# zhiqiangdon/pose-adv-aug

Hardware: AMD Instinct MI355X
Metric: images/sec, 2-stack HG 256x256 bs=24 per GPU, full training step (higher is better)
Workload: dtype bf16; 1 GPU; BASELINE configs[1]: 2-stack hourglass chan 256, bs=24/GPU, 256x256 MPII-shape synthetic frames (720x1280 uint8 resident in HBM), on-device HumanAug warp, heat-map MSE, RMSprop, PCKh; global_batch=24, parallelism=dp1, ranks_seen=1, devices_seen=1

## Files before the change

### include/poseadv.h

```cpp
#ifndef POSEADV_H
#define POSEADV_H
#include <stddef.h>
#include <stdint.h>
#ifdef __cplusplus
extern "C" {
#endif

const char* pa_last_error(void);
int pa_version(void);
int pa_dtype(void);
float pa_grad_scale(void);


int pa_gaussian_heatmap(const double* pts, float* out, int B, int J, int H, int W, void* stream);

int pa_weighted_l2(const float* pred, const float* gt, const float* weight, size_t n, float* loss, void* stream);
int pa_weighted_l2_grad(const float* pred, const float* gt, const float* weight, size_t n, const float* gout_dev,
                        float* dpred, void* stream);

int pa_get_preds(const float* maps, int B, int J, int H, int W, float* preds, float* maxval, void* stream);

int pa_final_preds(const float* maps, const float* center, const float* scale, const float* rot,
                   int B, int J, int H, int W, float* out, float* scratch_preds, void* stream);

// ... 157 lines not shown

int pa_asn_forward(pa_net* asn, pa_net* pose, int train, float* logits_scale, float* logits_rot);
const float* pa_asn_probs(const pa_net* asn);
int pa_asn_backward(pa_net* asn, pa_net* pose, const float* target_scale, const float* target_rot, float* loss);
int pa_asn_set_log_eps(pa_net* asn, float eps);

int pa_asn_forward_masks(pa_net* asn, pa_net* pose, int train, float* mask_logits);
int pa_asn_backward_masks(pa_net* asn, pa_net* pose, const float* dlogits);
int pa_hg_set_dropout_masks(pa_net* net, const float* masks);

int pa_hg_accuracy(pa_net* net, int stack, const int32_t* idxs, int nidx, float* acc, float* scratch);

int pa_hg_pckh(pa_net* net, int stack, const float* center, const float* scale, const float* rot, const float* gt_pts,
               const float* norm, const int32_t* idxs, int nidx, float* acc, float* person, float* scratch);

int pa_net_meters_async(pa_net* net, int on);

#define PA_PROF_CLASSES 12
int pa_net_profile_begin(pa_net* net);
int pa_net_profile_report(pa_net* net, double* out_host, int cap_classes, int* n_classes);
int pa_net_profile_classes(const pa_net* net, int32_t* out_host, int cap);
int pa_net_set_fin_prologue(pa_net* net, int max_rows);
int pa_net_set_pool_route(pa_net* net, int on);
int pa_net_design_bytes(const pa_net* net, double* out_host);
int pa_copy_probe(void* dst, const void* src, size_t bytes, void* stream);
int pa_copy_probe_form(void* dst, const void* src, size_t bytes, int form, void* stream);
int pa_conv2d_time(int mode, int variant, int B, int Cin, int Cout, int H, int W, int k, int iters, void* ws, float* ms_out, void* stream);
int pa_conv_plan_describe(int B, int H, int W, int Cin, int Cout, int taps, int in_mode, int add1_mode, int add2_mode, int ep_mode,
                          int ep2_mode, int fin_rows, int flags, int cus, int* out, int cap);
int pa_conv_launch_log(int* out, int cap);

int pa_net_set_multi_stream(pa_net* net, int on);

int pa_hg_debug_tensor(pa_net* net, const char* which, int grad, float* out, int* shape4);

int pa_asn_debug_tensor(pa_net* net, const char* which, int grad, float* out, int* shape4);

#ifdef __cplusplus
}
#endif
#endif
```

### pose_adv_aug_amd/_lib.py

```python
import ctypes as C
import os

import torch

_HERE = os.path.dirname(os.path.abspath(__file__))
DTYPE = os.environ.get('POSEADV_DTYPE', 'bf16').lower()
if DTYPE not in ('bf16', 'fp16'):
    raise ValueError('POSEADV_DTYPE must be bf16 or fp16')
LIB_PATH = os.path.join(_HERE, 'libposeadv_hip.so' if DTYPE == 'bf16' else 'libposeadv_hip_fp16.so')


def set_dtype(name):
    global DTYPE, LIB_PATH
    name = name.lower()
    if name not in ('bf16', 'fp16'):
        raise ValueError('dtype must be bf16 or fp16')
    if _lib is not None and name != DTYPE:
        raise PoseAdvError('the %s library is already loaded in this process' % DTYPE)
    DTYPE = name
    LIB_PATH = os.path.join(_HERE, 'libposeadv_hip.so' if name == 'bf16' else 'libposeadv_hip_fp16.so')


def act_dtype():
    return torch.bfloat16 if DTYPE == 'bf16' else torch.float16
# ... 115 lines not shown
    'pa_hg_bucket_wait': (_i, [_vp, _i, _vp]),
    'pa_hg_train_step': (_i, [_vp, _vp, _vp, _i, _i, _vp]),
    'pa_hg_set_loss_total': (_i, [_vp, _vp]),
    'pa_hg_set_heat_grads': (_i, [_vp, C.POINTER(_vp), _i]),
    'pa_hg_set_image_grad': (_i, [_vp, _vp, _i]),
    'pa_stem_dgrad_workspace_bytes': (_sz, [_i, _i, _i]),
    'pa_stem_dgrad': (_i, [_vp, _vp, _vp, _i, _i, _i, _i, _vp, _vp]),
    'pa_hg_accuracy': (_i, [_vp, _i, _vp, _i, _vp, _vp]),
    'pa_hg_forward_half': (_i, [_vp, _vp, _vp, _i]),
    'pa_asn_forward': (_i, [_vp, _vp, _i, _vp, _vp]),
    'pa_asn_probs': (_vp, [_vp]),
    'pa_asn_backward': (_i, [_vp, _vp, _vp, _vp, _vp]),
    'pa_asn_set_log_eps': (_i, [_vp, _f]),
    'pa_hg_pckh': (_i, [_vp, _i, _vp, _vp, _vp, _vp, _vp, _vp, _i, _vp, _vp, _vp]),
    'pa_net_meters_async': (_i, [_vp, _i]),
    'pa_net_profile_begin': (_i, [_vp]),
    'pa_net_profile_report': (_i, [_vp, C.POINTER(C.c_double), _i, C.POINTER(_i)]),
    'pa_net_design_bytes': (_i, [_vp, C.POINTER(C.c_double)]),
    'pa_copy_probe': (_i, [_vp, _vp, _sz, _vp]),
    'pa_copy_probe_form': (_i, [_vp, _vp, _sz, _i, _vp]),
    'pa_params_csr': (_i, [_vp, _i, _vp, _vp]),
    'pa_net_set_fin_prologue': (_i, [_vp, _i]),
    'pa_net_set_pool_route': (_i, [_vp, _i]),
    'pa_wgrad_group_workspace_bytes': (_sz, [_vp, _i]),
    'pa_wgrad_group': (_i, [_vp, _i, _i, _vp, _vp]),
    'pa_conv2d_time': (_i, [_i] * 9 + [_vp, C.POINTER(C.c_float), _vp]),
    'pa_conv_plan_describe': (_i, [_i] * 14 + [C.POINTER(_i), _i]),
    'pa_conv_launch_log': (_i, [C.POINTER(_i), _i]),
    'pa_net_profile_classes': (_i, [_vp, C.POINTER(C.c_int32), _i]),
    'pa_net_set_multi_stream': (_i, [_vp, _i]),
    'pa_hg_debug_tensor': (_i, [_vp, C.c_char_p, _i, _vp, C.POINTER(_i)]),
    'pa_asn_debug_tensor': (_i, [_vp, C.c_char_p, _i, _vp, C.POINTER(_i)]),
}

EXPORTS = sorted(_PROTOS)


def lib():
    global _lib
    if _lib is None:
        if not os.path.isfile(LIB_PATH):
            raise PoseAdvError('%s not found: run `python -c "import __graft_entry__ as g; g.build()"` '
                               '(there is no CPU fallback)' % LIB_PATH)
        try:
            l = C.CDLL(LIB_PATH)
        except OSError as e:
# ... 41 lines not shown
```

### pose_adv_aug_amd/csrc/api.hip

```cpp
#include "../../include/poseadv.h"
#include "net.h"
#include "warp_bwd.h"
#include "soft_argmax.h"
#include <stdio.h>
#include <string.h>
#include <new>
#include <string>

static thread_local char g_err[1024] = "";
void pa_set_error(const char* what, hipError_t e, const char* file, int line) {
    snprintf(g_err, sizeof g_err, "%s:%d: %s -> %s", file, line, what, hipGetErrorString(e));
}
void pa_set_error_msg(const char* msg) { snprintf(g_err, sizeof g_err, "%s", msg); }

struct pa_net { Net n; };
#define ST(s) reinterpret_cast<hipStream_t>(s)
#define TRY(x) do { int _r = (x); if (_r) { if (!g_err[0]) pa_set_error("kernel launch", (hipError_t)_r, __FILE__, __LINE__); return _r; } } while (0)
#define NEED_PTR(fn, p) do { if (!(p)) { pa_set_error_msg(fn ": " #p " is NULL"); return 1; } } while (0)
#define NEED_POS(fn, v) do { if ((v) < 1) { pa_set_error_msg(fn ": " #v " must be >= 1"); return 1; } } while (0)

extern "C" {

const char* pa_last_error(void) { return g_err; }
float pa_grad_scale(void) { return PA_GRAD_SCALE; }
// ... 874 lines not shown
}

int pa_net_profile_begin(pa_net* net) { net->n.prof.used = 0; net->n.prof.on = true; return 0; }
int pa_net_profile_report(pa_net* net, double* out, int cap_classes, int* n_classes) {
    net->n.prof.on = false;
    double full[PA_PROF_NCLS * 4];
    int r = net->n.prof.report(full);
    if (r) { pa_set_error("profile report", (hipError_t)r, __FILE__, __LINE__); return r; }
    for (int c = 0; c < PA_PROF_NCLS && c < cap_classes; ++c)
        for (int j = 0; j < 4; ++j) out[c * 4 + j] = full[c * 4 + j];
    if (n_classes) *n_classes = PA_PROF_NCLS;
    return 0;
}
int pa_net_set_fin_prologue(pa_net* net, int max_rows) {
    net->n.fin_rows_max = max_rows < 0 ? 0 : (max_rows > PA_FIN_SMALL_ROWS ? PA_FIN_SMALL_ROWS : max_rows);
    net->n.release_graph();
    return 0;
}
int pa_net_set_pool_route(pa_net* net, int on) {
    net->n.pool_route = on ? 3 : 0;
    net->n.release_graph();
    return 0;
}
int pa_net_design_bytes(const pa_net* net, double* out) { out[0] = net->n.dbytes_rd; out[1] = net->n.dbytes_wr; return 0; }

int pa_net_profile_classes(const pa_net* net, int32_t* out, int cap) {
    const std::vector<int>& q = net->n.prof.last_seq;
    for (int i = 0; i < cap && i < (int)q.size(); ++i) out[i] = q[i];
    return (int)q.size();
}

int pa_net_set_multi_stream(pa_net* net, int on) {
    if (net->n.ensure_streams()) return 1;
    net->n.release_graph();
    net->n.multi_stream = on != 0 && net->n.side != nullptr;
    return 0;
}

static int debug_copy(Net& n, const Act& a, int grad, float* out, int* shape4, const char* who, const bf16* mat) {
    if (grad < 0 || grad > 4) { pa_set_error_msg((std::string(who) + ": grad must be 0 .. 4").c_str()); return 1; }
    if ((grad == 1 || grad == 3) && !a.grad) { pa_set_error_msg((std::string(who) + ": this tensor has no gradient buffer").c_str()); return 1; }
    if (grad == 4 && !mat) { pa_set_error_msg((std::string(who) + ": no stored BatchNorm-backward gradient of this tensor in this step").c_str()); return 1; }
    shape4[0] = a.B; shape4[1] = a.C; shape4[2] = a.H; shape4[3] = a.W;
    if (!out) return 0;
    const PaOperand src = grad == 0 ? n.op(a) : grad == 1 ? pa_plain(a.grad) : grad == 2 ? pa_plain(a.raw) : grad == 3 ? n.gradop(a) : pa_plain(mat);
    TRY(pa_launch_nhwc_bf16_to_nchw_f32(src, out, a.B, a.C, a.H, a.W, n.st));
// ... 97 lines not shown
```

### pose_adv_aug_amd/csrc/asn.hip

```cpp
#include "net.h"
#include <string.h>

#define TRY(x) do { int _r = (x); if (_r) return _r; } while (0)

static PaEpilogue ep_plain() { PaEpilogue e; memset(&e, 0, sizeof e); e.mode = PA_OUT_PLAIN; return e; }

__global__ void pooladd_fwd_kernel(PaOperand hi, PaOperand lo, bf16* out, int B, int H, int W, int C) {
    const int CG = C / 8;
    const size_t total = (size_t)B * H * W * CG;
    for (size_t t = (size_t)blockIdx.x * blockDim.x + threadIdx.x; t < total; t += (size_t)gridDim.x * blockDim.x) {
        const int cg = (int)(t % CG);
        const size_t p = t / CG;
        const int x = (int)(p % W);
        const size_t q = p / W;
        const int y = (int)(q % H), b = (int)(q / H);
        const int c = cg * 8;
        float m[8], v[8];
#pragma unroll
        for (int k = 0; k < 4; ++k) {
            const size_t idx = (((size_t)b * 2 * H + 2 * y + (k >> 1)) * 2 * W + 2 * x + (k & 1)) * C + c;
            pa_read8(hi, idx, c, v);
#pragma unroll
            for (int j = 0; j < 8; ++j) m[j] = (k == 0) ? v[j] : fmaxf(m[j], v[j]);
        }
// ... 136 lines not shown
    for (int k = 0; k < 5; ++k) asn_in[k].declare(*this, names[k], chan, chan, false);
    char buf[32];
    for (int k = 0; k < 4; ++k) { snprintf(buf, sizeof buf, "merge%d.", k + 1); asn_merge[k].declare(*this, buf, chan, chan, false); }
    for (int k = 0; k < 3; ++k) { snprintf(buf, sizeof buf, "deep_merge.%d.", k); asn_deep[k].declare(*this, buf, chan, chan, false); }
    if (asn_dropout) {
        p_oc_w = add_param("out_conv.weight", {1, chan, 1, 1});
        p_oc_b = add_param("out_conv.bias", {1});
    } else {
        p_fcs_w = add_param("fc_scale.weight", {scale_num, chan});
        p_fcs_b = add_param("fc_scale.bias", {scale_num});
        p_fcr_w = add_param("fc_rotation.weight", {rot_num, chan});
        p_fcr_b = add_param("fc_rotation.bias", {rot_num});
    }
    n_params = (n_params + 3) & ~(size_t)3;
}

size_t Net::layout_asn(char* base) {
    Arena a; a.base = base;
    loss_dev = a.get<float>(64);
    a.take(0);
    stats_arena = base ? reinterpret_cast<float*>(base) : nullptr;
    stats_arena_floats = a.off / sizeof(float);
    prep_jobs = a.get<PaPrepJob>(convs.size());
    red_jobs = a.get<PaWgradReduceJob>(convs.size());
    bneval_jobs = a.get<PaBnEvalJob>(bns.size());
    const int H = res / 4;
    for (int k = 0; k < 5; ++k) asn_in[k].layout(*this, a, B, H >> k, H >> k, true);
    for (int k = 0; k < 4; ++k) {
        asn_pa[k] = new_act(a, B, H >> (k + 1), H >> (k + 1), chan, nullptr, true);
        asn_merge[k].layout(*this, a, B, H >> (k + 1), H >> (k + 1), true);
    }
    for (int k = 0; k < 3; ++k) asn_deep[k].layout(*this, a, B, H >> 4, H >> 4, true);
    asn_feat = a.get<float>((size_t)B * chan);
    asn_logits = a.get<float>((size_t)B * (asn_dropout ? 16 : scale_num + rot_num));
    asn_probs = a.get<float>((size_t)B * (scale_num + rot_num));
    asn_dlogits = a.get<float>((size_t)B * (scale_num + rot_num));
    a.take(0);
    return a.off;
}

int Net::forward_half(const float* img_nchw, const bf16* img4_in, bool train) {
    train_bn = train;
    TRY(ensure_streams());
    TRY(begin_step());
    if (!train) TRY(pa_launch_bn_eval(bneval_jobs, n_bneval, eps, st));
    const bf16* image = img4_in ? img4_in : img4;
// ... 110 lines not shown
```

### pose_adv_aug_amd/csrc/elementwise.hip

```cpp
#include "common.h"
#include "kernels.h"
#ifndef PA_ELT_PRIO
#define PA_ELT_PRIO 2
#endif
#define PA_SET_ELT_PRIO() do { if (PA_ELT_PRIO > 0) __builtin_amdgcn_s_setprio(PA_ELT_PRIO); } while (0)
#include "bn_fin.h"
#include <type_traits>
#include <hip/hip_ext.h>
static unsigned fin_launch_flags() { return pa_tuning().fin_anyorder ? hipExtAnyOrderLaunch : 0u; }
template <class... P, class... A>
static void fin_launch(void (*kernel)(P...), dim3 grid, int threads, hipStream_t st, A... args) {
    if (fin_launch_flags()) hipExtLaunchKernelGGL(kernel, grid, dim3(threads), 0, st, nullptr, nullptr, fin_launch_flags(), static_cast<P>(args)...);
    else hipLaunchKernelGGL(kernel, grid, dim3(threads), 0, st, static_cast<P>(args)...);
}

template <class F>
static void fin_dispatch(F f) {
    f(std::integral_constant<int, 512>{}, std::integral_constant<int, 8>{});
}
template <int FT, int FC>
__device__ __forceinline__ void reduce_partial_rows(const float* part, int rows, int C, int c0, float (*sums)[2]) {
    constexpr int SL = FT / FC;
    __shared__ __attribute__((aligned(16))) float red[SL][FC + 1][2];
    const int cl = threadIdx.x % FC, sl = threadIdx.x / FC;
// ... 1135 lines not shown
        const bool ok = n < j.Cout && c < j.Cin;
        const float* src = j.w + ((size_t)n * j.Cin + c) * j.taps;
        for (int tap = 0; tap < j.taps; ++tap) {
            const bf16 v = (bf16)(ok ? src[tap] : 0.f);
            j.wf[((size_t)n * j.taps + tap) * j.pad_cin + c] = v;
            tile[tap][tn][tc] = v;
        }
        __syncthreads();
        if (j.wb) {
            for (int tap = 0; tap < j.taps; ++tap)
                j.wb[((size_t)(c0 + tn) * j.taps + (j.taps - 1 - tap)) * j.pad_cout + n0 + tc] = tile[tap][tc][tn];
        }
        __syncthreads();
    }
}

int pa_launch_weight_prep(const PaPrepJob* jobs_dev, int njobs, int max_elems, hipStream_t st) {
    if (njobs <= 0) return 0;
    (void)max_elems;
    hipLaunchKernelGGL(weight_prep_kernel, dim3(32, njobs), dim3(1024), 0, st, jobs_dev);
    return (int)hipGetLastError();
}

__global__ void nchw_to_nhwc4_kernel(const float* src, bf16* dst, int B, int H, int W) {
    const size_t total = (size_t)B * H * W;
    for (size_t p = (size_t)blockIdx.x * blockDim.x + threadIdx.x; p < total; p += (size_t)gridDim.x * blockDim.x) {
        size_t hw = (size_t)H * W;
        size_t b = p / hw, r = p - b * hw;
        bf16x4 o;
        o[0] = (bf16)src[(b * 3 + 0) * hw + r];
        o[1] = (bf16)src[(b * 3 + 1) * hw + r];
        o[2] = (bf16)src[(b * 3 + 2) * hw + r];
        o[3] = (bf16)0.f;
        *reinterpret_cast<bf16x4*>(dst + p * 4) = o;
    }
}

int pa_launch_nchw_to_nhwc4(const float* src, bf16* dst, int B, int H, int W, hipStream_t st) {
    size_t total = (size_t)B * H * W;
    const int blocks = pa_grid_for(total, 256, 4096);
    hipLaunchKernelGGL(nchw_to_nhwc4_kernel, dim3(blocks), dim3(256), 0, st, src, dst, B, H, W);
    return (int)hipGetLastError();
}

__global__ void nhwc_to_nchw_f32_kernel(const float* src, float* dst, int B, int H, int W, int C) {
    const size_t total = (size_t)B * C * H * W;
// ... 137 lines not shown
```

### pose_adv_aug_amd/csrc/kernels.h

```cpp
#pragma once
#include "common.h"
#include "bn_fin.h"
#include "launch_plan.h"
#include "wgrad_plan.h"
#include "conv_plan.h"

struct PaConvArgs {
    PaOperand in;
    const bf16* w;
    const float* bias;
    PaOperand add1;
    PaOperand add2;
    PaEpilogue ep;
    bf16* out;
    int B, H, W, Cin, Cout, taps;
    bf16* dz_out;
    PaBnFin fin;
    int low_prio;
    int dbg;
    int xcd;
    PaEpilogue ep2;
    bf16* out2;
};
int pa_conv_cus();
// ... 68 lines not shown
    int B, Hm, Wm, layout;
    float scale;
};
int pa_launch_stem_dgrad(const PaStemDgradArgs& a, hipStream_t st);
int pa_launch_stem_pack(const float* w, bf16* wf, hipStream_t st);

int pa_launch_rmsprop(float* p, const float* g, float* v, size_t n, float lr, float alpha, float eps, float gscale, int* state, hipStream_t st);
struct PaRmspropOpts { float lr, alpha, eps, mom, wd; };
int pa_launch_rmsprop_opts(const PaRmspropOpts& o, bool centered, float* p, const float* g, float* v, float* buf, float* ga, size_t n,
                           float gscale, const float* clip_coef, int* state, hipStream_t st);
size_t pa_grad_norm_workspace_size(size_t n);
int pa_launch_grad_norm(const float* g, size_t n, float gscale, float max_norm, void* workspace, float* out2, hipStream_t st);
struct PaAdamOpts { float lr, beta1, beta2, eps, wd, c_dec, om_b1, om_b2; };
struct PaAdamState { int flag, skipped, step, reserved; float bc1, bc2, step_size, bc2s; };
int pa_launch_adam(const PaAdamOpts& o, bool amsgrad, int decay, float* p, const float* g, float* m, float* v, float* vmax, size_t n,
                   float gscale, const float* clip_coef, PaAdamState* state, hipStream_t st);
int pa_adam_read_steps(const PaAdamState* state, long long* steps, long long* skipped, hipStream_t st);
int pa_launch_adam_set_steps(PaAdamState* state, int steps, hipStream_t st);
int pa_launch_loss_out(float* acc, float* keep, float* out, float* total, int n, hipStream_t st);
int pa_launch_copy16(void* dst, const void* src, size_t bytes, hipStream_t st, int form = 0);
int pa_rmsprop_skipped(const int* state, long long* out, hipStream_t st);
struct PaPrepJob { const float* w; bf16* wf; bf16* wb; int Cout, Cin, taps, pad_cout, pad_cin; };
int pa_launch_weight_prep(const PaPrepJob* jobs_dev, int njobs, int max_elems, hipStream_t st);

int pa_launch_nchw_to_nhwc4(const float* src, bf16* dst, int B, int H, int W, hipStream_t st);
int pa_launch_nhwc_to_nchw_f32(const float* src, float* dst, int B, int H, int W, int C, hipStream_t st);
int pa_launch_nchw_f32_to_nhwc_bf16(const float* src, bf16* dst, int B, int C, int H, int W, hipStream_t st);
int pa_launch_nhwc_bf16_to_nchw_f32(const PaOperand& src, float* dst, int B, int C, int H, int W, hipStream_t st);

int pa_launch_cell_mask(const PaOperand& x, const float* mask, const PaEpilogue& ep, bf16* out, int B, int H, int W, int C,
                        hipStream_t st);
int pa_launch_ep_apply(const PaOperand& g, const PaEpilogue& ep, bf16* out, size_t M, int C, hipStream_t st, int* stat_rows = nullptr);
int pa_launch_fill(float* p, float v, size_t n, hipStream_t st);
```

### pose_adv_aug_amd/csrc/net.h

```cpp
#pragma once
#include <string>
#include <vector>
#include "common.h"
#include "kernels.h"
#include "pose_ops.h"

struct Arena {
    char* base = nullptr;
    size_t off = 0;
    void* take(size_t bytes) {
        off = (off + 255) & ~(size_t)255;
        void* p = base ? base + off : nullptr;
        off += bytes;
        return p;
    }
    template <typename T> T* get(size_t n) { return reinterpret_cast<T*>(take(n * sizeof(T))); }
};

struct TensorInfo {
    std::string name;
    int shape[4];
    int ndim;
    size_t offset;
    size_t numel;
// ... 105 lines not shown
    int decode(Net& n);
    int bwd(Net& n, const Act& in, const PaOperand& extra0);
    const Act& out() const { return merged[0]; }
    bool low_fusable(const Net& n, int k) const;
};

struct Net {
    int stacks = 2, modules = 1, chan = 256, classes = 16, B = 0, res = 256;
    bool is_agent = false;
    std::vector<TensorInfo> tensors;
    size_t n_params = 0, n_buffers = 0;
    std::vector<ConvLayer*> convs;
    std::vector<BNLayer*> bns;
    float *params = nullptr, *grads = nullptr, *buffers = nullptr;
    char* workspace = nullptr;
    size_t workspace_bytes = 0;
    float *stats_arena = nullptr;
    size_t stats_arena_floats = 0;
    float* loss_dev = nullptr;
    float* loss_keep = nullptr;
    float* loss_total_out = nullptr;
    bool loss_self_clearing = false;
    PaPrepJob* prep_jobs = nullptr; int n_prep = 0, prep_max = 0;
    PaWgradReduceJob* red_jobs = nullptr; int n_red = 0, red_max = 0;
    PaBnEvalJob* bneval_jobs = nullptr; int n_bneval = 0;
    hipStream_t st = nullptr;
    hipStream_t side = nullptr;
    hipEvent_t ev_fork[4], ev_join[4];
    bool streams_ready = false, multi_stream = !pa_tuning().single_stream;
    hipStream_t wstream = nullptr;
    bool wgrads_aside() const { return multi_stream && wstream != nullptr; }
    hipEvent_t ev_w[16]; int ev_w_next = 0;
    hipEvent_t ev_wdone;
    struct PendingWgrad { PaWgradArgs a; int cls; double bytes, flops; bool stem; int job_wgs; ConvLayer* c; };
    std::vector<PendingWgrad> pending_wgrads;
    bool on_side = false;
    int flush_wgrads();
    int launch_pending_wgrads();
    std::vector<int> red_stash; int red_stash_mx = 0, red_stash_flushes = 0;
    int flush_red_stash(hipStream_t ws);
    void drop_wgrads();
    int ensure_streams();
    void release_streams();
    int fork_to(int k);
    int record_join(int k);
    int wait_join(int k);
// ... 60 lines not shown
                 bf16* out, BNLayer* bn_after, BNLayer* pending_in = nullptr, bool defer_after = false);
    int conv_dgrad(ConvLayer& c, const PaOperand& dy, int B, int H, int W, const PaOperand& add1, const PaOperand& add2,
                   const PaEpilogue& ep, bf16* out, bf16* dz_out = nullptr, bool* dz_done = nullptr, BNLayer* pending_in = nullptr,
                   const Act* low = nullptr, bool* low_done = nullptr,
                   const PaEpilogue* pool_in_ep = nullptr);
    int fin_rows_max = pa_tuning().fin_prologue > PA_FIN_SMALL_ROWS ? PA_FIN_SMALL_ROWS : pa_tuning().fin_prologue;
    int pool_route = pa_tuning().pool_route;
    bool maps_on = false;
    unsigned char* stem_map = nullptr; bf16* stem_xmax = nullptr;
    bool stem_map_written = false, stem_routed = false;
    bool stem_route_ok();
    int fill_stem_grad();
    int fin_mask = pa_tuning().fin_mask;
    bool fin_consumer_ok(const ConvLayer& c, int B, int H, int W, bool dgrad) const;
    PaBnFin fin_fwd(const BNLayer& b, int M) const;
    PaBnFin fin_bwd(const BNLayer& b, int M) const;
    int finish_grad_or_defer(const Act& a, bool defer);
    int finish_grad2_or_defer(const Act& a, bool defer_a, const Act& b, bool defer_b);
    bool x3_fin_ok(const Residual& r, const Act& in) const;
    bool x3_fin_ok(const Chain& c, const Act& in) const { return x3_fin_ok(c.tail(), c.tail_in(in)); }
    int conv_wgrad(ConvLayer& c, const PaOperand& dy, const PaOperand& x, int B, int H, int W);

    int prepare_weights();
    int begin_step();
    const bf16* cur_image = nullptr;
    int forward_pose(const float* img_nchw, const bf16* img4_in, const double* pts, bool train, float* loss_out_dev);
    int forward_pose_body(const float* img_nchw, const bf16* img4_in, const double* pts, bool train, float* loss_out_dev);
    int backward_pose();
    int backward_stack(int i);
    int backward_stem();
    hipEvent_t ev_bucket[16], ev_bucket_main = nullptr; bool bucket_events = false;
    int mark_bucket(int stack);
    int reduce_grads();
    int forward_half(const float* img_nchw, const bf16* img4_in, bool train);

    int scale_num = 7, rot_num = 7;
    Residual asn_in[5];
    Residual asn_merge[4];
    Residual asn_deep[3];
    size_t p_fcs_w = 0, p_fcs_b = 0, p_fcr_w = 0, p_fcr_b = 0;
    Act asn_pa[4];
    float *asn_feat = nullptr, *asn_logits = nullptr, *asn_probs = nullptr, *asn_dlogits = nullptr;
    void declare_asn();
    size_t layout_asn(char* base);
    int asn_forward(Net& pose, bool train, float* logits_s, float* logits_r);
    float asn_log_eps = 1e-7f;
// ... 12 lines not shown
```

### pose_adv_aug_amd/csrc/net.hip

```cpp
#include "net.h"
#include <stdio.h>
#include <string.h>

static int ablate() { return pa_tuning().ablate; }
static int ablate_h() { return pa_tuning().ablate_h; }
#define TRY(x) do { int _r = (x); if (_r) return _r; } while (0)

PaOperand pa_plain(const bf16* p) { PaOperand o; o.p = p; o.q = nullptr; o.k0 = o.k1 = o.k2 = nullptr; o.map = nullptr; o.mode = PA_LD_PLAIN; return o; }
PaOperand pa_none() { PaOperand o; o.p = o.q = nullptr; o.k0 = o.k1 = o.k2 = nullptr; o.map = nullptr; o.mode = PA_LD_NONE; return o; }
static PaEpilogue ep_plain() { PaEpilogue e; memset(&e, 0, sizeof e); e.mode = PA_OUT_PLAIN; return e; }
static int round64(int v) { return (v + 63) / 64 * 64; }

size_t Net::add_param(const std::string& name, std::initializer_list<int> shape) {
    TensorInfo t; t.name = name; t.ndim = (int)shape.size(); t.is_buffer = 0;
    size_t n = 1; int i = 0;
    for (int s : shape) { t.shape[i++] = s; n *= (size_t)s; }
    for (; i < 4; ++i) t.shape[i] = 1;
    n_params = (n_params + 3) & ~(size_t)3;
    t.offset = n_params; t.numel = n;
    n_params += n;
    tensors.push_back(t);
    return t.offset;
}

size_t Net::add_buffer(const std::string& name, int C) {
// ... 132 lines not shown
        down[k].layout(n, a, B, H >> (k + 1), W >> (k + 1), need_grad);
        poolgrad[k] = need_grad ? a.get<bf16>((size_t)B * (H >> k) * (W >> k) * C) : nullptr;
        poolmap[k] = need_grad ? a.get<unsigned char>(pooled[k].numel()) : nullptr;
    }
    neck.layout(n, a, B, H >> 4, W >> 4, need_grad);
    for (int k = 3; k >= 0; --k) {
        up[k].layout(n, a, B, H >> (k + 1), W >> (k + 1), need_grad, 4);
        merged[k] = n.new_act(a, B, H >> k, W >> k, C, nullptr, need_grad);
    }
    for (int k = 0; k < 4; ++k) skipm[k] = n.new_act(a, B, H >> k, W >> k, C, nullptr, need_grad);
    neckm = n.new_act(a, B, H >> 4, W >> 4, C, nullptr, need_grad);
}

size_t Net::layout_all(char* base) {
    Arena a; a.base = base;
    size_t zero_begin = a.off;
    loss_dev = a.get<float>(64);
    a.take(0);
    stats_arena = base ? reinterpret_cast<float*>(base + zero_begin) : nullptr;
    stats_arena_floats = (a.off - zero_begin) / sizeof(float);
    loss_keep = a.get<float>(64);
    loss_self_clearing = true;
    prep_jobs = a.get<PaPrepJob>(convs.size());
    red_jobs = a.get<PaWgradReduceJob>(convs.size());
    bneval_jobs = a.get<PaBnEvalJob>(bns.size());

    const int H2 = res / 2, H4 = res / 4;
    img4 = a.get<bf16>((size_t)B * res * res * 4);
    pts_dev = a.get<double>((size_t)B * classes * 2);
    layout_conv(stem_conv, a, B * H2 * H2);
    layout_bn(stem_bn, a, B * H2 * H2);
    a0 = new_act(a, B, H2, H2, 64, &stem_bn, true);
    res1.layout(*this, a, B, H2, H2, true);
    pool0 = new_act(a, B, H4, H4, 128, nullptr, true);
    stem_map = a.get<unsigned char>(pool0.numel());
    stem_xmax = a.get<bf16>(pool0.numel());
    res2.layout(*this, a, B, H4, H4, true);
    res3.layout(*this, a, B, H4, H4, true);
    lin_out.resize(stacks); xin.resize(stacks); heat.resize(stacks); heat_peak.resize(stacks); heat_peak_valid.assign(stacks, 0); heat64.resize(stacks); dheat64.resize(stacks);
    dheat_in.resize(stacks); forth_tmp.resize(stacks); lgrad_tmp.resize(stacks);
    const int M = B * H4 * H4;
    for (int i = 0; i < stacks; ++i) {
        hg[i].layout(*this, a, B, H4, H4, true);
        post[i].layout(*this, a, B, H4, H4, true);
        layout_conv(lin[i], a, M, H4, H4); layout_bn(lin_bn[i], a, M);
        lin_out[i] = new_act(a, B, H4, H4, chan, &lin_bn[i], true);
// ... 17 lines not shown

int Net::upload_tables() {
    std::vector<PaPrepJob> pj; std::vector<PaWgradReduceJob> rj; std::vector<PaBnEvalJob> bj;
    prep_max = 0; red_max = 0;
    for (ConvLayer* c : convs) {
        PaPrepJob p; p.w = params + c->p_w; p.wf = c->wf; p.wb = c->wb; p.Cout = c->Cout; p.Cin = c->Cin;
        p.taps = c->k == 7 ? 49 : c->taps(); p.pad_cout = c->pcout; p.pad_cin = c->pcin;
        pj.push_back(p);
        int pe = c->pcout * (c->k == 7 ? 256 : c->taps() * c->pcin);
        if (pe > prep_max) prep_max = pe;
        if (c->k == 7) continue;
        PaWgradReduceJob r; r.part = c->part; r.dst = grads + c->p_w; r.dbpart = c->dbpart; r.dbdst = grads + c->p_b;
        r.Cout = c->pcout; r.Cin = c->pcin; r.taps = c->taps(); r.splits = c->splits; r.real_cout = c->Cout; r.real_cin = c->Cin;
        c->red_index = (int)rj.size();
        rj.push_back(r);
        int re = c->Cout * c->Cin * c->taps() + c->Cout;
        if (re > red_max) red_max = re;
    }
    for (BNLayer* b : bns) {
        PaBnEvalJob j; j.gamma = params + b->p_gamma; j.beta = params + b->p_beta; j.rmean = buffers + b->b_rmean;
        j.rvar = buffers + b->b_rvar; j.scale = b->scale; j.shift = b->shift; j.C = b->C;
        bj.push_back(j);
    }
    n_prep = (int)pj.size(); n_red = (int)rj.size(); n_bneval = (int)bj.size();
    PA_CHECK(hipMemcpyAsync(prep_jobs, pj.data(), pj.size() * sizeof(PaPrepJob), hipMemcpyHostToDevice, st));
    PA_CHECK(hipMemcpyAsync(red_jobs, rj.data(), rj.size() * sizeof(PaWgradReduceJob), hipMemcpyHostToDevice, st));
    PA_CHECK(hipMemcpyAsync(bneval_jobs, bj.data(), bj.size() * sizeof(PaBnEvalJob), hipMemcpyHostToDevice, st));
    PA_CHECK(hipStreamSynchronize(st));
    return 0;
}

ProfEntry* Prof::begin(int cls, double bytes, double flops, hipStream_t st) {
    if (!on) return nullptr;
    if (used == entries.size()) {
        ProfEntry e; e.cls = 0; e.bytes = e.flops = 0;
        if (hipEventCreate(&e.e0) != hipSuccess || hipEventCreate(&e.e1) != hipSuccess) return nullptr;
        entries.push_back(e);
    }
    ProfEntry* e = &entries[used++];
    e->cls = cls; e->bytes = bytes; e->flops = flops;
    hipEventRecord(e->e0, st);
    return e;
}

void Prof::end(ProfEntry* e, hipStream_t st) { if (e) hipEventRecord(e->e1, st); }

int Prof::report(double* out) {
// ... 553 lines not shown
}
void Net::release_streams() {
    release_graph();
    if (bucket_events) { for (int i = 0; i < 16; ++i) (void)hipEventDestroy(ev_bucket[i]); (void)hipEventDestroy(ev_bucket_main); bucket_events = false; }
    if (mstream) { (void)hipStreamSynchronize(mstream); (void)hipStreamDestroy(mstream); (void)hipEventDestroy(ev_mfork); (void)hipEventDestroy(ev_meter); mstream = nullptr; meter_pending = false; }
    if (side) {
        (void)hipStreamSynchronize(side); (void)hipStreamDestroy(side); side = nullptr;
        for (int k = 0; k < 4; ++k) { (void)hipEventDestroy(ev_fork[k]); (void)hipEventDestroy(ev_join[k]); }
    }
    if (wstream) {
        (void)hipStreamSynchronize(wstream); (void)hipStreamDestroy(wstream); wstream = nullptr;
        for (int i = 0; i < 16; ++i) (void)hipEventDestroy(ev_w[i]);
        (void)hipEventDestroy(ev_wdone);
    }
    for (ProfEntry& e : prof.entries) { (void)hipEventDestroy(e.e0); (void)hipEventDestroy(e.e1); }
    prof.entries.clear(); prof.used = 0;
    streams_ready = false;
}
int Net::fork_to(int k) { PA_CHECK(hipEventRecord(ev_fork[k], st)); PA_CHECK(hipStreamWaitEvent(side, ev_fork[k], 0)); return 0; }
int Net::record_join(int k) { PA_CHECK(hipEventRecord(ev_join[k], side)); return 0; }
int Net::wait_join(int k) { PA_CHECK(hipStreamWaitEvent(st, ev_join[k], 0)); return 0; }

int Net::prepare_weights() { return pa_launch_weight_prep(prep_jobs, n_prep, prep_max, st); }

int Net::begin_step() {
    dbytes_rd = dbytes_wr = 0;
    if (!loss_self_clearing) PA_CHECK(hipMemsetAsync(stats_arena, 0, stats_arena_floats * sizeof(float), st));
    return 0;
}

int Net::meter_stream(hipStream_t* out) {
    *out = st;
    if (!meters_async || !multi_stream) return join_meters();
    if (!mstream) {
        PA_CHECK(hipStreamCreateWithFlags(&mstream, hipStreamNonBlocking));
        PA_CHECK(hipEventCreateWithFlags(&ev_mfork, hipEventDisableTiming));
        PA_CHECK(hipEventCreateWithFlags(&ev_meter, hipEventDisableTiming));
    }
    PA_CHECK(hipEventRecord(ev_mfork, st));
    PA_CHECK(hipStreamWaitEvent(mstream, ev_mfork, 0));
    *out = mstream;
    return 0;
}
int Net::meter_done(hipStream_t ms) {
    if (ms == st) return 0;
    PA_CHECK(hipEventRecord(ev_meter, ms));
// ... 224 lines not shown
```

### pose_adv_aug_amd/csrc/tuning.h

```cpp
#pragma once
#include <stdlib.h>

#define PA_TUNING_TABLE(X)                                                                                                           \
                                                                      \
    X(conv1_old,        "PA_CONV1_OLD",        0,   "1x1 convolutions on the generic kernel (no row-tile kernel, no fused upsample-add gradient)") \
    X(conv3_old,        "PA_CONV3_OLD",        0,   "3x3 convolutions on the generic kernel (no halo-tile kernel)")                 \
    X(wgrad_old,        "PA_WGRAD_OLD",        0,   "weight gradients on the generic kernel (no tile kernel, stem included)")       \
    X(stem_wgrad_old,   "PA_STEM_WGRAD_OLD",   0,   "the stem's weight gradient on the generic kernel")                            \
    X(eltwise_old,      "PA_ELTWISE_OLD",      0,   "pooling / upsample-add / cell-mask launches in their first, unvectorised form") \
    X(conv3_nosmall,    "PA_CONV3_NOSMALL",    0,   "no 8 x 8 / 4 x 4 halo tiles: the small maps go to the generic kernel")        \
    X(igemm_oneshot,    "PA_IGEMM_ONESHOT",    1,   "0: the small 1x1 layers on the K-stepping generic kernel instead of the one-shot one") \
    X(no_dz3,           "PA_NO_DZ3",           0,   "conv3's data gradient does not store dz3 (its readers recompute it)")         \
    X(no_dz2,           "PA_NO_DZ2",           0,   "conv2's data gradient does not store dz2")                                    \
    X(epi_bwd_direct,   "PA_EPI_BWD_DIRECT",   0,   "direct (no LDS) BatchNorm-backward epilogue wherever an instance carries both") \
    X(conv3_noxcd,      "PA_CONV3_NOXCD",      0,   "3x3 tiles in launch order instead of one contiguous range per XCD")           \
    X(wg_group,         "PA_WG_GROUP",         1,   "0: one launch per weight gradient instead of group launches")                 \
    X(wg_red_in_group,  "PA_WG_RED_IN_GROUP",  1,   "0: slab reductions as launches of their own instead of inside the next group launch") \
    X(wgrad_anyorder,   "PA_WGRAD_ANYORDER",   1,   "0: ungrouped weight gradients of one flush as ordinary in-order launches")    \
    X(wgrad_nopipe,     "PA_WGRAD_NOPIPE",     0,   "plain instead of pipelined tile weight gradients")                            \
    X(upadd_fuse,       "PA_UPADD_FUSE",       1,   "0: the upsample-add backward's low-resolution half as a launch of its own")   \
    X(upadd_split,      "PA_UPADD_SPLIT",      1,   "0: both halves of the upsample-add backward in one launch on the main stream") \
    X(pool_route,       "PA_POOL_ROUTE",       3,   "pool gradients through the forward pools' arg-max maps: bit 0 the hourglass pools, bit 1 the stem's pool (0: a pool backward launch each)") \
    X(fin_prologue,     "PA_FIN_PROLOGUE",     128, "most partial rows a consumer finalizes in its prologue (0: always a finalize launch; at most 128)") \
    X(fin_mask,         "PA_FIN_MASK",         7,   "which finalizes may ride in a consumer: 1 forward x1 / x2, 2 backward x2, 4 backward x3") \
    X(single_stream,    "PA_SINGLE_STREAM",    0,   "everything on the caller's stream")                                           \
    X(no_wstream,       "PA_NO_WSTREAM",       0,   "side streams, but the weight gradients on the stream that produced their operands") \
    X(stem_on_main,     "PA_STEM_ON_MAIN",     1,   "0: the stem's weight gradient on the weight-gradient stream")                 \
                                                              \
    X(wgrad_wgs1,       "PA_WGRAD_WGS1",       256, "workgroup target of a 1x1 tile weight gradient launched alone")               \
    X(wgrad_wgs9,       "PA_WGRAD_WGS9",       256, "the same for 3x3")                                                            \
    X(wgrad_min1,       "PA_WGRAD_MIN1",       3,   "fewest 128-pixel tiles for which a 1x1 weight gradient takes the tile kernel") \
    X(wg_group_wgs1,    "PA_WG_GROUP_WGS1",    64,  "workgroup budget of a 1x1 job of a group launch")                             \
    X(wg_group_wgs9,    "PA_WG_GROUP_WGS9",    64,  "the same for 3x3")                                                            \
    X(wg_group_minper1, "PA_WG_GROUP_MINPER1", 2,   "fewest tiles per workgroup of a 1x1 job")                                     \
    X(wg_group_minper9, "PA_WG_GROUP_MINPER9", 4,   "the same for 3x3")                                                            \
    X(wg_group_cap,     "PA_WG_GROUP_CAP",     256, "most workgroups of one group launch")                                         \
    X(wg_red_wgs,       "PA_WG_RED_WGS",       256, "workgroups of the slab reduction inside a group launch")                      \
    X(wreduce_lag,      "PA_WREDUCE_LAG",      2,   "flushes whose slabs wait in the stash before they are summed")                \
    X(stem_splits,      "PA_STEM_SPLITS",      512, "splits (slabs) of the stem's weight gradient")                                \
    X(wgrad_tile1,      "PA_WGRAD_TILE1",      0,   "generic 1x1 weight gradient: forced tile variant (0: by shape)")              \
    X(wgrad_tile9,      "PA_WGRAD_TILE9",      0,   "the same for 3x3")                                                            \
    X(wgrad_blocks,     "PA_WGRAD_BLOCKS",     0,   "generic weight gradient: forced split count (0: by shape)")                   \
                                                                                    \
    X(ablate,           "PA_ABLATE",           0,   "INSTRUMENT, wrong results: mask of launch classes that are skipped (net.hip)") \
    X(ablate_h,         "PA_ABLATE_H",         8,   "INSTRUMENT: largest map height the low-resolution bits of PA_ABLATE skip")    \
// ... 29 lines not shown
```

### pose_adv_aug_amd/models/asn_stacked_hg.py

```python
import ctypes as C
import math
from collections import OrderedDict

import numpy as np
import torch

from .. import _lib
from .._lib import lib, check, ptr, stream, require_gpu, PoseAdvError


class _HipModule(object):

    def __init__(self):
        self.training = True
        self._nets = {}
        self._table = None
        self.flat_params = self.flat_grads = self.flat_buffers = None
        self._nbt = 0
        self._weights_dirty = True

    def _create(self, B):
        raise NotImplementedError

    def _read_table(self, h):
# ... 29 lines not shown
            self._nets[B] = (h, ws)
            if len(self._nets) == 1:
                self._weights_dirty = False
        h, _ = self._nets[B]
        if self._weights_dirty:
            for hh, _ in self._nets.values():
                check(lib().pa_net_prepare_weights(hh), 'pa_net_prepare_weights')
            self._weights_dirty = False
        return h

    def _ensure_table(self):
        if self._table is None:
            self._net(self.default_batch)

    def __del__(self):
        try:
            for h, _ in self._nets.values():
                lib().pa_net_destroy(h)
        except Exception:
            pass

    def weights_changed(self):
        self._weights_dirty = True

    def named_parameters(self):
        self._ensure_table()
        for name, shape, off, numel, kind in self._table:
            if kind == 0:
                yield name, self.flat_params[off:off + numel].view(shape)

    def parameters(self):
        return [p for _, p in self.named_parameters()]

    def named_grads(self):
        self._ensure_table()
        for name, shape, off, numel, kind in self._table:
            if kind == 0:
                yield name, self.flat_grads[off:off + numel].view(shape)

    def state_dict(self, prefix=''):
        self._ensure_table()
        sd = OrderedDict()
        for name, shape, off, numel, kind in self._table:
            if kind == 0:
                sd[prefix + name] = self.flat_params[off:off + numel].view(shape)
            elif kind == 1:
# ... 399 lines not shown
```

### pose_adv_aug_amd/utils/optim.py

```python
import ctypes as C
import os

import torch
import torch.distributed as dist

from .. import _lib
from .._lib import lib, check, ptr, stream


def _dist_on():
    return dist.is_available() and dist.is_initialized() and (dist.get_world_size() > 1 or os.environ.get('POSEADV_FORCE_DIST') == '1')


def optim_options(opt):
    clip = float(getattr(opt, 'clip_grad_norm', 0) or 0)
    return dict(momentum=float(getattr(opt, 'momentum', 0) or 0), weight_decay=float(getattr(opt, 'weight_decay', 0) or 0),
                centered=bool(getattr(opt, 'centered', 0)), max_grad_norm=clip if clip > 0 else None)


class _FlatOptimizer(object):
    def _attach(self, net, max_grad_norm, overlap):
        if max_grad_norm is not None and not max_grad_norm > 0:
            raise ValueError('max_grad_norm must be > 0 (None: no clipping)')
        self.net = net
# ... 78 lines not shown
class RMSprop(_FlatOptimizer):
    def __init__(self, net, lr=2.5e-4, alpha=0.99, eps=1e-8, momentum=0, weight_decay=0, centered=False, max_grad_norm=None, overlap=False):
        if momentum < 0 or weight_decay < 0:
            raise ValueError('momentum and weight_decay must be >= 0')
        self._attach(net, max_grad_norm, overlap)
        self.param_groups = [{'lr': lr, 'alpha': alpha, 'eps': eps, 'momentum': momentum, 'weight_decay': weight_decay, 'centered': bool(centered)}]
        self.square_avg = torch.zeros_like(net.flat_params)
        self.momentum_buffer = self.grad_avg = None
        self._ensure_state(self.param_groups[0])
        self._skip_state = torch.zeros(2, dtype=torch.int32, device=net.flat_params.device)
        self.steps = 0

    def _ensure_state(self, g):
        if g.get('momentum', 0) > 0 and self.momentum_buffer is None:
            self.momentum_buffer = torch.zeros_like(self.net.flat_params)
        if g.get('centered', False) and self.grad_avg is None:
            self.grad_avg = torch.zeros_like(self.net.flat_params)

    def step(self):
        g = self.param_groups[0]
        gscale = self._exchanged_gscale()
        n = self.net.flat_params.numel()
        mom, wd, centered = float(g.get('momentum', 0)), float(g.get('weight_decay', 0)), bool(g.get('centered', False))
        if mom == 0 and wd == 0 and not centered and self.max_grad_norm is None:
            check(lib().pa_rmsprop_step_state(ptr(self.net.flat_params), ptr(self.net.flat_grads), ptr(self.square_avg), n,
                                              float(g['lr']), float(g['alpha']), float(g['eps']), float(gscale), ptr(self._skip_state), stream()),
                  'pa_rmsprop_step_state')
        else:
            self._step_opts(g, mom, wd, centered, n, gscale)
        self.steps += 1
        self._weights_stepped()

    def _step_opts(self, g, mom, wd, centered, n, gscale):
        self._ensure_state(g)
        grads, coef = self.net.flat_grads, self._clip_coef(n, gscale)
        o = _lib.RmspropOpts(float(g['lr']), float(g['alpha']), float(g['eps']), mom, wd, int(centered))
        check(lib().pa_rmsprop_step_opts(C.byref(o), ptr(self.net.flat_params), ptr(grads), ptr(self.square_avg),
                                         ptr(self.momentum_buffer) if mom > 0 else None, ptr(self.grad_avg) if centered else None,
                                         n, float(gscale), coef, ptr(self._skip_state), stream()), 'pa_rmsprop_step_opts')

    def skipped_steps(self):
        n = C.c_longlong(0)
        check(lib().pa_rmsprop_skipped_steps_state(ptr(self._skip_state), C.byref(n), stream()), 'pa_rmsprop_skipped_steps_state')
        return int(n.value)

    def _option_state(self, g):
        self._ensure_state(g)
# ... 196 lines not shown
```

Before: 4242 images/sec.

## Fuse RMSprop optimizer step with bf16 weight re-pack into one launch

Adds a kernel that applies the RMSprop update to each conv's fp32 weights and writes the packed bf16 forward and backward weight layouts in the same pass. Non-conv parameter ranges are updated by extra blocks of the same launch. This removes a separate full-buffer optimizer launch followed by a weight-prep launch that re-reads the fresh weights. The cost is more complex indexing, a per-net range table, and extra prepare calls for other cached batch-size nets.

```diff
diff --git a/include/poseadv.h b/include/poseadv.h
--- a/include/poseadv.h
+++ b/include/poseadv.h
@@ -203,6 +203,9 @@
 int pa_net_profile_classes(const pa_net* net, int32_t* out_host, int cap);
 int pa_net_set_fin_prologue(pa_net* net, int max_rows);
 int pa_net_set_pool_route(pa_net* net, int on);
+int pa_net_rmsprop_step(pa_net* net, float* square_avg, float lr, float alpha, float eps, float gscale, int32_t* state, void* stream);
+int pa_net_set_fused_step(pa_net* net, int on);
+int pa_net_fused_step(const pa_net* net);
 int pa_net_design_bytes(const pa_net* net, double* out_host);
 int pa_copy_probe(void* dst, const void* src, size_t bytes, void* stream);
 int pa_copy_probe_form(void* dst, const void* src, size_t bytes, int form, void* stream);
diff --git a/pose_adv_aug_amd/_lib.py b/pose_adv_aug_amd/_lib.py
--- a/pose_adv_aug_amd/_lib.py
+++ b/pose_adv_aug_amd/_lib.py
@@ -161,6 +161,9 @@
     'pa_params_csr': (_i, [_vp, _i, _vp, _vp]),
     'pa_net_set_fin_prologue': (_i, [_vp, _i]),
     'pa_net_set_pool_route': (_i, [_vp, _i]),
+    'pa_net_rmsprop_step': (_i, [_vp, _vp, _f, _f, _f, _f, _vp, _vp]),
+    'pa_net_set_fused_step': (_i, [_vp, _i]),
+    'pa_net_fused_step': (_i, [_vp]),
     'pa_wgrad_group_workspace_bytes': (_sz, [_vp, _i]),
     'pa_wgrad_group': (_i, [_vp, _i, _i, _vp, _vp]),
     'pa_conv2d_time': (_i, [_i] * 9 + [_vp, C.POINTER(C.c_float), _vp]),
diff --git a/pose_adv_aug_amd/csrc/api.hip b/pose_adv_aug_amd/csrc/api.hip
--- a/pose_adv_aug_amd/csrc/api.hip
+++ b/pose_adv_aug_amd/csrc/api.hip
@@ -920,6 +920,14 @@
     net->n.release_graph();
     return 0;
 }
+int pa_net_set_fused_step(pa_net* net, int on) { net->n.fused_step = on ? 1 : 0; return 0; }
+int pa_net_fused_step(const pa_net* net) { return net->n.fused_step && net->n.ranges_ready ? 1 : 0; }
+int pa_net_rmsprop_step(pa_net* net, float* square_avg, float lr, float alpha, float eps, float gscale, int32_t* state, void* s) {
+    g_err[0] = 0;
+    if (!net || !square_avg || !state) { pa_set_error_msg("pa_net_rmsprop_step: net, square_avg or state is NULL"); return 1; }
+    TRY(net->n.rmsprop_step(square_avg, lr, alpha, eps, gscale, state, ST(s)));
+    return 0;
+}
 int pa_net_design_bytes(const pa_net* net, double* out) { out[0] = net->n.dbytes_rd; out[1] = net->n.dbytes_wr; return 0; }
 
 int pa_net_profile_classes(const pa_net* net, int32_t* out, int cap) {
diff --git a/pose_adv_aug_amd/csrc/asn.hip b/pose_adv_aug_amd/csrc/asn.hip
--- a/pose_adv_aug_amd/csrc/asn.hip
+++ b/pose_adv_aug_amd/csrc/asn.hip
@@ -182,6 +182,7 @@
     stats_arena = base ? reinterpret_cast<float*>(base) : nullptr;
     stats_arena_floats = a.off / sizeof(float);
     prep_jobs = a.get<PaPrepJob>(convs.size());
+    step_ranges = a.get<PaStepRange>(convs.size() + 1);
     red_jobs = a.get<PaWgradReduceJob>(convs.size());
     bneval_jobs = a.get<PaBnEvalJob>(bns.size());
     const int H = res / 4;
diff --git a/pose_adv_aug_amd/csrc/elementwise.hip b/pose_adv_aug_amd/csrc/elementwise.hip
--- a/pose_adv_aug_amd/csrc/elementwise.hip
+++ b/pose_adv_aug_amd/csrc/elementwise.hip
@@ -1181,6 +1181,146 @@
     return (int)hipGetLastError();
 }
 
+__device__ __forceinline__ float rmsprop_v_fused(float v, float gr, float alpha) {
+#pragma clang fp contract(off)
+    const float t = ((1.f - alpha) * gr) * gr;
+    return __builtin_fmaf(alpha, v, t);
+}
+__device__ __forceinline__ float rmsprop_p_fused(float p, float v, float gr, float lr, float eps) {
+#pragma clang fp contract(off)
+    const float q = gr / (sqrtf(v) + eps);
+    float r = __builtin_fmaf(-lr, q, p);
+    asm volatile("" : "+v"(r));
+    return r;
+}
+template <int TAPS, int CW, bool EDGE>
+__device__ __forceinline__ void rmsprop_prep_row(const PaPrepJob& j, size_t r0, int n, int c0, int tn, int tc, bf16* tile, float* p,
+                                                 const float* g, float* v, float lr, float alpha, float eps, float gscale) {
+    constexpr int K = CW * TAPS, S = 32 * K + 2;
+    if (EDGE) {
+#pragma unroll 1
+        for (int e = tc; e < 32 * K; e += 32) {
+            float pn = 0.f;
+            if (n < j.Cout && c0 + e / TAPS < j.Cin) {
+                const float gr = g[r0 + e] * gscale;
+                const float vn = rmsprop_v_fused(v[r0 + e], gr, alpha);
+                pn = rmsprop_p_fused(p[r0 + e], vn, gr, lr, eps);
+                v[r0 + e] = vn;
+                p[r0 + e] = pn;
+            }
+            tile[tn * S + e] = (bf16)pn;
+        }
+        return;
+    }
+    float pp[K], gg[K], vv[K];
+#pragma unroll
+    for (int k = 0; k < K; ++k) {
+        pp[k] = p[r0 + tc + 32 * k];
+        gg[k] = g[r0 + tc + 32 * k];
+        vv[k] = v[r0 + tc + 32 * k];
+    }
+#pragma unroll
+    for (int k = 0; k < K; ++k) {
+        const int e = tc + 32 * k;
+        const float gr = gg[k] * gscale;
+        const float vn = rmsprop_v_fused(vv[k], gr, alpha);
+        const float pn = rmsprop_p_fused(pp[k], vn, gr, lr, eps);
+        v[r0 + e] = vn;
+        p[r0 + e] = pn;
+        tile[tn * S + e] = (bf16)pn;
+    }
+}
+
+template <int TAPS, int CW>
+__device__ __forceinline__ void rmsprop_prep_tiles(const PaPrepJob& j, size_t base, bf16* tile, float* p, const float* g, float* v,
+                                                   float lr, float alpha, float eps, float gscale) {
+    constexpr int K = CW * TAPS, S = 32 * K + 2, TC = 32 * CW;
+    const int tn = threadIdx.x >> 5, tc = threadIdx.x & 31;
+    const int tiles_c = j.pad_cin / TC, ntiles = (j.pad_cout / 32) * tiles_c;
+    for (int t = blockIdx.x; t < ntiles; t += gridDim.x) {
+        const int n0 = (t / tiles_c) * 32, c0 = (t % tiles_c) * TC;
+        const int n = n0 + tn;
+        const size_t r0 = base + ((size_t)n * j.Cin + c0) * TAPS;
+        if (n0 + 32 <= j.Cout && c0 + TC <= j.Cin) rmsprop_prep_row<TAPS, CW, false>(j, r0, n, c0, tn, tc, tile, p, g, v, lr, alpha, eps, gscale);
+        else rmsprop_prep_row<TAPS, CW, true>(j, r0, n, c0, tn, tc, tile, p, g, v, lr, alpha, eps, gscale);
+        __syncthreads();
+#pragma unroll
+        for (int tap = 0; tap < TAPS; ++tap)
+#pragma unroll
+            for (int w = 0; w < CW; ++w)
+                j.wf[((size_t)n * TAPS + tap) * j.pad_cin + c0 + tc + 32 * w] = tile[tn * S + (tc + 32 * w) * TAPS + tap];
+        if (j.wb) {
+#pragma unroll
+            for (int tap = 0; tap < TAPS; ++tap)
+#pragma unroll
+                for (int w = 0; w < CW; ++w)
+                    j.wb[((size_t)(c0 + tn + 32 * w) * TAPS + (TAPS - 1 - tap)) * j.pad_cout + n0 + tc] = tile[tc * S + (tn + 32 * w) * TAPS + tap];
+        }
+        __syncthreads();
+    }
+}
+
+__global__ __launch_bounds__(1024) __attribute__((amdgpu_waves_per_eu(8))) void rmsprop_prep_kernel(const PaPrepJob* jobs, int njobs, const PaStepRange* ranges, int nranges, float* p,
+                                                             const float* g, float* v, float lr, float alpha, float eps, float gscale, int* state) {
+#ifdef PA_FP16
+    int* gs = state ? state : g_grad_state;
+    if (gs[0]) {
+        if (blockIdx.x == 0 && blockIdx.y == 0 && threadIdx.x == 0) gs[1] += 1;
+        return;
+    }
+#endif
+    if ((int)blockIdx.y >= njobs) {
+        const int ri = ((int)blockIdx.y - njobs) * (int)gridDim.x + (int)blockIdx.x;
+        if (ri >= nranges) return;
+        const PaStepRange r = ranges[ri];
+        for (size_t i = r.lo + threadIdx.x; i < r.hi; i += blockDim.x) {
+            const float gr = g[i] * gscale;
+            const float vn = rmsprop_v_fused(v[i], gr, alpha);
+            v[i] = vn;
+            p[i] = rmsprop_p_fused(p[i], vn, gr, lr, eps);
+        }
+        return;
+    }
+    const PaPrepJob j = jobs[blockIdx.y];
+    const size_t base = (size_t)(j.w - p);
+    if (j.taps == 49) {
+        const int total = j.pad_cout * 256;
+        for (int e = blockIdx.x * blockDim.x + threadIdx.x; e < total; e += gridDim.x * blockDim.x) {
+            int n = e >> 8, k = e & 255;
+            int ky = k >> 5, kx = (k & 31) >> 2, c = k & 3;
+            float pn = 0.f;
+            if (n < j.Cout && ky < 7 && kx < 7 && c < j.Cin) {
+                const size_t i = base + ((size_t)(n * j.Cin + c) * 7 + ky) * 7 + kx;
+                const float gr = g[i] * gscale;
+                const float vn = rmsprop_v_fused(v[i], gr, alpha);
+                pn = rmsprop_p_fused(p[i], vn, gr, lr, eps);
+                v[i] = vn;
+                p[i] = pn;
+            }
+            j.wf[e] = (bf16)pn;
+        }
+        return;
+    }
+    __shared__ bf16 tile[32 * (32 * 9 + 2)];
+    if (j.taps == 1) rmsprop_prep_tiles<1, 2>(j, base, tile, p, g, v, lr, alpha, eps, gscale);
+    else rmsprop_prep_tiles<9, 1>(j, base, tile, p, g, v, lr, alpha, eps, gscale);
+}
+
+int pa_launch_rmsprop_prep(const PaPrepJob* jobs_dev, int njobs, const PaStepRange* ranges_dev, int nranges, float* p, const float* g, float* v,
+                           size_t n, float lr, float alpha, float eps, float gscale, int* state, hipStream_t st) {
+    if (njobs + nranges <= 0) return 0;
+#ifdef PA_FP16
+    const int blocks = pa_grid_for(n / 4, 256, 2048);
+    hipLaunchKernelGGL(grad_check_reset_kernel, dim3(1), dim3(1), 0, st, state);
+    hipLaunchKernelGGL(grad_check_kernel, dim3(blocks), dim3(256), 0, st, g, n, state);
+#else
+    (void)n;
+#endif
+    hipLaunchKernelGGL(rmsprop_prep_kernel, dim3(32, njobs + (nranges + 31) / 32), dim3(1024), 0, st, jobs_dev, njobs, ranges_dev, nranges, p, g, v,
+                       lr, alpha, eps, gscale, state);
+    return (int)hipGetLastError();
+}
+
 __global__ void nchw_to_nhwc4_kernel(const float* src, bf16* dst, int B, int H, int W) {
     const size_t total = (size_t)B * H * W;
     for (size_t p = (size_t)blockIdx.x * blockDim.x + threadIdx.x; p < total; p += (size_t)gridDim.x * blockDim.x) {
diff --git a/pose_adv_aug_amd/csrc/kernels.h b/pose_adv_aug_amd/csrc/kernels.h
--- a/pose_adv_aug_amd/csrc/kernels.h
+++ b/pose_adv_aug_amd/csrc/kernels.h
@@ -114,6 +114,9 @@
 int pa_rmsprop_skipped(const int* state, long long* out, hipStream_t st);
 struct PaPrepJob { const float* w; bf16* wf; bf16* wb; int Cout, Cin, taps, pad_cout, pad_cin; };
 int pa_launch_weight_prep(const PaPrepJob* jobs_dev, int njobs, int max_elems, hipStream_t st);
+struct PaStepRange { size_t lo, hi; };
+int pa_launch_rmsprop_prep(const PaPrepJob* jobs_dev, int njobs, const PaStepRange* ranges_dev, int nranges, float* p, const float* g, float* v,
+                           size_t n, float lr, float alpha, float eps, float gscale, int* state, hipStream_t st);
 
 int pa_launch_nchw_to_nhwc4(const float* src, bf16* dst, int B, int H, int W, hipStream_t st);
 int pa_launch_nhwc_to_nchw_f32(const float* src, float* dst, int B, int H, int W, int C, hipStream_t st);
diff --git a/pose_adv_aug_amd/csrc/net.h b/pose_adv_aug_amd/csrc/net.h
--- a/pose_adv_aug_amd/csrc/net.h
+++ b/pose_adv_aug_amd/csrc/net.h
@@ -151,6 +151,9 @@
     float* loss_total_out = nullptr;
     bool loss_self_clearing = false;
     PaPrepJob* prep_jobs = nullptr; int n_prep = 0, prep_max = 0;
+    PaStepRange* step_ranges = nullptr; int n_ranges = 0;
+    bool ranges_ready = false;
+    int fused_step = pa_tuning().fused_step;
     PaWgradReduceJob* red_jobs = nullptr; int n_red = 0, red_max = 0;
     PaBnEvalJob* bneval_jobs = nullptr; int n_bneval = 0;
     hipStream_t st = nullptr;
@@ -257,6 +260,7 @@
     int conv_wgrad(ConvLayer& c, const PaOperand& dy, const PaOperand& x, int B, int H, int W);
 
     int prepare_weights();
+    int rmsprop_step(float* v, float lr, float alpha, float eps, float gscale, int* state, hipStream_t s);
     int begin_step();
     const bf16* cur_image = nullptr;
     int forward_pose(const float* img_nchw, const bf16* img4_in, const double* pts, bool train, float* loss_out_dev);
diff --git a/pose_adv_aug_amd/csrc/net.hip b/pose_adv_aug_amd/csrc/net.hip
--- a/pose_adv_aug_amd/csrc/net.hip
+++ b/pose_adv_aug_amd/csrc/net.hip
@@ -1,6 +1,8 @@
 #include "net.h"
 #include <stdio.h>
 #include <string.h>
+#include <algorithm>
+#include <utility>
 
 static int ablate() { return pa_tuning().ablate; }
 static int ablate_h() { return pa_tuning().ablate_h; }
@@ -179,6 +181,7 @@
     loss_keep = a.get<float>(64);
     loss_self_clearing = true;
     prep_jobs = a.get<PaPrepJob>(convs.size());
+    step_ranges = a.get<PaStepRange>(convs.size() + 1);
     red_jobs = a.get<PaWgradReduceJob>(convs.size());
     bneval_jobs = a.get<PaBnEvalJob>(bns.size());
 
@@ -242,7 +245,35 @@
         j.rvar = buffers + b->b_rvar; j.scale = b->scale; j.shift = b->shift; j.C = b->C;
         bj.push_back(j);
     }
+    std::stable_partition(pj.begin(), pj.end(), [](const PaPrepJob& q) { return q.taps == 9; });
     n_prep = (int)pj.size(); n_red = (int)rj.size(); n_bneval = (int)bj.size();
+    n_ranges = 0; ranges_ready = false;
+    if (step_ranges) {
+        std::vector<std::pair<size_t, size_t>> w;
+        bool ok = true;
+        for (ConvLayer* c : convs) {
+            w.push_back({c->p_w, c->p_w + (size_t)c->Cout * c->Cin * c->k * c->k});
+            if (c->k != 1 && c->k != 3 && c->k != 7) ok = false;
+        }
+        std::sort(w.begin(), w.end());
+        std::vector<PaStepRange> sr;
+        size_t pos = 0, covered = 0;
+        for (const auto& q : w) {
+            if (q.first < pos || q.second > n_params) { ok = false; break; }
+            if (q.first > pos) { sr.push_back({pos, q.first}); covered += q.first - pos; }
+            covered += q.second - q.first;
+            pos = q.second;
+        }
+        if (ok && pos < n_params) { sr.push_back({pos, n_params}); covered += n_params - pos; }
+        if (!ok || covered != n_params || sr.size() > convs.size() + 1) {
+            pa_set_error_msg("upload_tables: the conv weights and the ranges between them do not tile the parameter buffer");
+            return 1;
+        }
+        n_ranges = (int)sr.size();
+        if (n_ranges) PA_CHECK(hipMemcpyAsync(step_ranges, sr.data(), sr.size() * sizeof(PaStepRange), hipMemcpyHostToDevice, st));
+        PA_CHECK(hipStreamSynchronize(st));
+        ranges_ready = true;
+    }
     PA_CHECK(hipMemcpyAsync(prep_jobs, pj.data(), pj.size() * sizeof(PaPrepJob), hipMemcpyHostToDevice, st));
     PA_CHECK(hipMemcpyAsync(red_jobs, rj.data(), rj.size() * sizeof(PaWgradReduceJob), hipMemcpyHostToDevice, st));
     PA_CHECK(hipMemcpyAsync(bneval_jobs, bj.data(), bj.size() * sizeof(PaBnEvalJob), hipMemcpyHostToDevice, st));
@@ -842,6 +873,14 @@
 int Net::wait_join(int k) { PA_CHECK(hipStreamWaitEvent(st, ev_join[k], 0)); return 0; }
 
 int Net::prepare_weights() { return pa_launch_weight_prep(prep_jobs, n_prep, prep_max, st); }
+
+int Net::rmsprop_step(float* v, float lr, float alpha, float eps, float gscale, int* state, hipStream_t s) {
+    if (!params || !grads || !ranges_ready) { pa_set_error_msg("rmsprop_step: the net is not bound"); return 1; }
+    if (fused_step)
+        return pa_launch_rmsprop_prep(prep_jobs, n_prep, step_ranges, n_ranges, params, grads, v, n_params, lr, alpha, eps, gscale, state, s);
+    TRY(pa_launch_rmsprop(params, grads, v, n_params, lr, alpha, eps, gscale, state, s));
+    return pa_launch_weight_prep(prep_jobs, n_prep, prep_max, s);
+}
 
 int Net::begin_step() {
     dbytes_rd = dbytes_wr = 0;
diff --git a/pose_adv_aug_amd/csrc/tuning.h b/pose_adv_aug_amd/csrc/tuning.h
--- a/pose_adv_aug_amd/csrc/tuning.h
+++ b/pose_adv_aug_amd/csrc/tuning.h
@@ -21,6 +21,7 @@
     X(upadd_fuse,       "PA_UPADD_FUSE",       1,   "0: the upsample-add backward's low-resolution half as a launch of its own")   \
     X(upadd_split,      "PA_UPADD_SPLIT",      1,   "0: both halves of the upsample-add backward in one launch on the main stream") \
     X(pool_route,       "PA_POOL_ROUTE",       3,   "pool gradients through the forward pools' arg-max maps: bit 0 the hourglass pools, bit 1 the stem's pool (0: a pool backward launch each)") \
+    X(fused_step,       "PA_FUSED_STEP",       1,   "0: the reference recipe's optimizer step and the weight re-pack as two launches instead of one") \
     X(fin_prologue,     "PA_FIN_PROLOGUE",     128, "most partial rows a consumer finalizes in its prologue (0: always a finalize launch; at most 128)") \
     X(fin_mask,         "PA_FIN_MASK",         7,   "which finalizes may ride in a consumer: 1 forward x1 / x2, 2 backward x2, 4 backward x3") \
     X(single_stream,    "PA_SINGLE_STREAM",    0,   "everything on the caller's stream")                                           \
diff --git a/pose_adv_aug_amd/models/asn_stacked_hg.py b/pose_adv_aug_amd/models/asn_stacked_hg.py
--- a/pose_adv_aug_amd/models/asn_stacked_hg.py
+++ b/pose_adv_aug_amd/models/asn_stacked_hg.py
@@ -75,6 +75,12 @@
 
     def weights_changed(self):
         self._weights_dirty = True
+
+    def _weights_packed(self, h):
+        for hh, _ in self._nets.values():
+            if hh != h:
+                check(lib().pa_net_prepare_weights(hh), 'pa_net_prepare_weights')
+        self._weights_dirty = False
 
     def named_parameters(self):
         self._ensure_table()
diff --git a/pose_adv_aug_amd/utils/optim.py b/pose_adv_aug_amd/utils/optim.py
--- a/pose_adv_aug_amd/utils/optim.py
+++ b/pose_adv_aug_amd/utils/optim.py
@@ -124,7 +124,15 @@
         gscale = self._exchanged_gscale()
         n = self.net.flat_params.numel()
         mom, wd, centered = float(g.get('momentum', 0)), float(g.get('weight_decay', 0)), bool(g.get('centered', False))
-        if mom == 0 and wd == 0 and not centered and self.max_grad_norm is None:
+        plain = mom == 0 and wd == 0 and not centered and self.max_grad_norm is None
+        h = self.net._net(self.net._last_B or self.net.default_batch) if plain else None
+        if h and lib().pa_net_fused_step(h) == 1:
+            check(lib().pa_net_rmsprop_step(h, ptr(self.square_avg), float(g['lr']), float(g['alpha']), float(g['eps']), float(gscale),
+                                            ptr(self._skip_state), stream()), 'pa_net_rmsprop_step')
+            self.steps += 1
+            self.net._weights_packed(h)
+            return
+        if plain:
             check(lib().pa_rmsprop_step_state(ptr(self.net.flat_params), ptr(self.net.flat_grads), ptr(self.square_avg), n,
                                               float(g['lr']), float(g['alpha']), float(g['eps']), float(gscale), ptr(self._skip_state), stream()),
                   'pa_rmsprop_step_state')
```

New measurement: 4261 images/sec (median of 6 runs). Within noise of the previous version (+0.4%).
